# emiliofidalgo/liodom

Hardware: AMD Instinct MI355X
Metric: scans/sec (64×1800 cloud, prev_frames=20) at 1 GPU; pose RMSE vs CPU ref (higher is better)
Workload: dtype f64

## Files before the change

liodom_amd/api.py:

```python
import ctypes as C
import hashlib
import os
import subprocess

import numpy as np

_HERE = os.path.dirname(os.path.abspath(__file__))
_ROOT = os.path.dirname(_HERE)
_LIB = os.path.join(_HERE, "lib", "libliodom_hip.so")
_HASH = _LIB + ".srchash"
_BUILD_INFO = {"rebuilt": None, "source_hash": None}
_SRC = [os.path.join(_HERE, "csrc", f) for f in ("liodom_hip.hip", "liodom_kernels.h", "kernels_extract.h", "kernels_sync.h",
                                                  "kernels_compact.h", "kernels_knn.h", "kernels_knn8.h", "kernels_lm.h", "kernels_rebuild.h",
                                                  "kernels_filter.h", "kernels_cov.h", "kernels_state.h", "liodom_math.h", "wave_ops.h",
                                                  "liodom_map.h", "liodom_map_host.h")] + [
    os.path.join(_ROOT, "include", "liodom_hip.h")]

HIPCC_FLAGS = ["--offload-arch=gfx950", "-O3", "-std=c++17", "-ffp-contract=off", "-fPIC", "-shared",
               "-Wno-unused-value"]


class LiodomError(RuntimeError):
    pass


def lib_path():
    return _LIB


def source_hash():
    h = hashlib.sha256()
    h.update(" ".join(HIPCC_FLAGS).encode())
    for p in _SRC:
        with open(p, "rb") as f:
            h.update(b"\0" + os.path.basename(p).encode() + b"\0" + f.read())
    return h.hexdigest()


def built_hash():
    try:
        with open(_HASH) as f:
            return f.read().strip()
    except OSError:
        return ""


def is_stale():
    return not os.path.exists(_LIB) or built_hash() != source_hash()


def build(force=False, verbose=False):
    import fcntl
    os.makedirs(os.path.dirname(_LIB), exist_ok=True)
    with open(_LIB + ".lock", "w") as lock:
        fcntl.flock(lock, fcntl.LOCK_EX)
        want = source_hash()
        if not force and os.path.exists(_LIB) and built_hash() == want:
            _BUILD_INFO.update(rebuilt=False, source_hash=want)
            return _LIB
        hipcc = "/opt/rocm/bin/hipcc" if os.path.exists("/opt/rocm/bin/hipcc") else "hipcc"
        tmp = _LIB + ".tmp.%d" % os.getpid()
        cmd = [hipcc] + HIPCC_FLAGS + ["-o", tmp, _SRC[0]]
        if verbose:
            print(" ".join(cmd))
        try:
            subprocess.check_call(cmd)
            os.replace(tmp, _LIB)
        finally:
            if os.path.exists(tmp):
                os.remove(tmp)
        with open(_HASH, "w") as f:
            f.write(want + "\n")
        _BUILD_INFO.update(rebuilt=True, source_hash=want)
    return _LIB


def build_info():
    return dict(_BUILD_INFO)


class Params(C.Structure):
    _fields_ = [
        ("min_range", C.c_double), ("max_range", C.c_double),
        ("lidar_type", C.c_int32), ("scan_lines", C.c_int32), ("scan_regions", C.c_int32),
        ("edges_per_region", C.c_int32),
        ("min_points_per_scan", C.c_uint64), ("local_map_size", C.c_uint64),
        ("save_results", C.c_int32),
        ("results_dir", C.c_char * 256), ("fixed_frame", C.c_char * 64), ("base_frame", C.c_char * 64),
        ("laser_frame", C.c_char * 64),
        ("use_imu", C.c_int32), ("filter_local_map", C.c_int32), ("mapping", C.c_int32), ("publish_tf", C.c_int32),
    ]


class Config(C.Structure):
    _fields_ = [
        ("device", C.c_int32), ("n_streams", C.c_int32), ("max_points", C.c_int32), ("max_width", C.c_int32),
        ("reserved1", C.c_int32), ("lm_apply_step_on_ftol", C.c_int32), ("pose_log_capacity", C.c_int32),
# ... 683 lines not shown
```

liodom_amd/csrc/kernels_lm.h:

```cpp
constexpr int kLmWaves = kLmThreads / 64;
__host__ __device__ __forceinline__ size_t lm_lds_bytes(int edge_cap) {
  return (size_t)((edge_cap + 3) & ~3) * sizeof(int);
}


__device__ int lm_compact_bits(const DevView& v, int s, int outer_it, int E, int* idx ) {
  const int lane = threadIdx.x & 63;
  const int Q = v.knn_queries;
  const int nb = (E + Q - 1) / Q;
  const int nwords = (nb + 3) >> 2;
  const unsigned int* mw = reinterpret_cast<const unsigned int*>(v.corr_mask + ((size_t)s * 2 + outer_it) * v.mask_stride);
  int run = 0;
  for (int w0 = 0; w0 < nwords; w0 += 64) {
    const int w = w0 + lane;
    unsigned int word = (w < nwords) ? mw[w] : 0u;
    const int pop = __popc(word);
    const int incl = wave_incl_scan_i32(pop);
    int o = run + incl - pop;
    while (word) {
      const int b = __ffs(word) - 1;
      word &= word - 1u;
      const int bit = w * 32 + b;
      idx[o++] = (bit >> 3) * Q + (bit & 7);
    }
// ... 245 lines not shown
  __hip_atomic_store((gu64*)(base + lane), ((unsigned long long)tag << 32) | word, __ATOMIC_RELAXED, __HIP_MEMORY_SCOPE_AGENT);
}

template <bool kList = false>
__global__ void k_imu_override(DevView v, int s0, int count) {
  const int i = blockIdx.x * blockDim.x + threadIdx.x;
  if (i >= count) return;
  const int s = stream_of_lane<kList>(v, s0, i);
  StreamState& st = v.state[s];
  if (!st.initialized) return;
  double odom[12], out[12], l2b[12], q[4];
#pragma unroll
  for (int k = 0; k < 12; k++) { odom[k] = st.odom[k]; l2b[k] = v.laser_to_base[k]; }
#pragma unroll
  for (int k = 0; k < 4; k++) q[k] = v.imu_q[(size_t)s * 4 + k];
  imu_override(odom, q, l2b, v.rotation_mode, out);
#pragma unroll
  for (int k = 0; k < 12; k++) st.odom[k] = out[k];
  quat_from_pose(out, v.rotation_mode, st.param_q);
  st.param_t[0] = out[3]; st.param_t[1] = out[7]; st.param_t[2] = out[11];
}

__device__ __forceinline__ void pose_cov_store(const DevView& v, int s, const StreamState& st, const LmState& lm, const double* acc, int nblocks, int tid) {
  const int j = tid - 64;
  if (j < 0 || j >= 21) return;
  PoseCovRaw* r = v.cov_raw + s;
  bool applied = lm.termination == LM_TERM_FUNC_TOL && lm.apply_on_ftol != 0;
  for (int k = 0; k < 4; k++) applied = applied && lm.q[k] == lm.cand_q[k];
  for (int k = 0; k < 3; k++) applied = applied && lm.t[k] == lm.cand_t[k];
  r->H[j] = applied ? acc[7 + j] : lm.H[j];
  if (j == 0) {
    r->scan_index = st.info.scan_index; r->n_res = nblocks; r->termination = lm.termination; r->has_solve = 1;
    r->cost = lm.cost;
  }
}

__device__ __forceinline__ void rebuild_beside_solve(const DevView& v, int s, StreamState& st, int eb, int outer_it, int block, int nblocks, unsigned int seq, int* sbase, int* sslot);

template <int kOuterIt, bool kChainMode, bool kList = false>
#ifndef LIODOM_LM_WAVES_PER_SIMD
#define LIODOM_LM_WAVES_PER_SIMD 1
#endif
__global__ __launch_bounds__(kLmThreads, LIODOM_LM_WAVES_PER_SIMD) void k_lm_solve(DevView v, int s0, int eb, unsigned int seq, unsigned int done_target) {
  constexpr int outer_it = kOuterIt;
  constexpr int chain = kChainMode ? 1 : 0;
  __shared__ double sh_pose2[2][12];
  __shared__ int sh_pi, sh_ci;
  __shared__ int sh_nmoved;
  __shared__ double sh_pred_s[20];
  __shared__ int sh_unapplied;
  __shared__ double sh_acc[kAccN];
  __shared__ LmState lm;
  __shared__ int sh_flag;
  __shared__ int sh_C;
  const int s = stream_of<kList>(v, s0, (int)blockIdx.y);
#if defined(LIODOM_CHAIN_PRIO)
  if (v.n_streams <= 4) __builtin_amdgcn_s_setprio(LIODOM_CHAIN_PRIO);
#endif
  const int G = v.lm_groups, gstride = G > 1 ? 8 : 1, bxl = (int)blockIdx.x;
  const bool is_solver = bxl < G * gstride && (bxl % gstride) == 0;
  const int g = is_solver ? bxl / gstride : G + (bxl < G * gstride ? bxl - (bxl / gstride + 1) : bxl - G);
  StreamState& st = v.state[s];
  __shared__ int sh_cnt[kMaxFrames + 1];
  OV_STAMP(v, bxl == 0 && threadIdx.x == 0, outer_it == 0 ? 0 : 3);
  if (seq && outer_it == 0 && bxl == 0 && threadIdx.x == 0) {
    typedef __attribute__((address_space(1))) unsigned int gu32;
    __hip_atomic_store((gu32*)(v.ov_flags + s), seq, __ATOMIC_RELAXED, __HIP_MEMORY_SCOPE_AGENT);
  }
  if (g >= G) {
    if (!v.early_rebuild || chain) return;
    __shared__ int sh_slot[kMaxFrames];
    rebuild_beside_solve(v, s, st, eb, outer_it, g - G, (int)gridDim.x - G, seq, sh_cnt, sh_slot);
    return;
  }
  __shared__ double sh_wsum[kLmWaves][32];
  __shared__ double sh_red[16][32];
  __shared__ double sh_x0[8];
  __shared__ double sh_prev[12];
  __shared__ int sh_fc;
  if (threadIdx.x < 4) sh_x0[threadIdx.x] = st.param_q[threadIdx.x];
  else if (threadIdx.x < 7) sh_x0[threadIdx.x] = st.param_t[threadIdx.x - 4];
  else if (threadIdx.x >= 64 && threadIdx.x < 76) sh_prev[threadIdx.x - 64] = st.prev_odom[threadIdx.x - 64];
  else if (threadIdx.x == 76) sh_fc = st.frame_count;
  __shared__ int sh_spec_at;
  if (threadIdx.x == 77) sh_spec_at = st.spec_eval[outer_it];
  __shared__ int sh_redo;
  if (threadIdx.x == 78) sh_redo = st.spec_redo[outer_it == 0 ? 1 : 0];
  extern __shared__ __attribute__((aligned(16))) int sh_idx[];
  const int tid = threadIdx.x;
  const bool prep = tid < kLmCtl;
  bool dead = false;
  if (chain && outer_it == 0) dead = !chain_wait_count(v.knn_done0 + s, done_target, &st.status);
  if (chain && outer_it == 0 && sh_redo) __builtin_amdgcn_fence(__ATOMIC_ACQUIRE, "agent");
  int E_in;
  if (chain && outer_it == 0) {
    typedef __attribute__((address_space(1))) unsigned int gu32;
    E_in = (int)__hip_atomic_load((gu32*)(v.edge_cnt + eb * 32 + s), __ATOMIC_RELAXED, __HIP_MEMORY_SCOPE_AGENT);
  } else {
    E_in = st.n_edges_buf[eb];
  }
  if (outer_it == 0 && tid == 0 && g == 0) {
    st.info.n_edges = E_in;
    st.info.map_points = st.n_search;
    for (int k = 0; k < 2; k++) {
      st.info.lm[k].iterations = 0; st.info.lm[k].accepted = 0; st.info.lm[k].termination = LM_TERM_NO_RESIDUALS;
      st.info.lm[k].pad = 0; st.info.lm[k].initial_cost = 0.0; st.info.lm[k].final_cost = 0.0;
    }
  }
  if (!st.initialized) {
    if (outer_it == 1 && g == 0) {
      if (seq) ov_wait_knn_done(v, s, seq, &st.status);
      if (tid == 0) st.append_raw = 1;
      __shared__ double sh_T0[12];
      if (tid < 12) sh_T0[tid] = st.odom[tid];
      __syncthreads();
      finalize_scan(v, s, st, sh_cnt, eb, true, 0, 0, sh_T0, 1, true, sh_prev, sh_fc);
      if (tid == 0) st.initialized = 1;
      if (v.cov_raw && tid == 64) {
        PoseCovRaw* r = v.cov_raw + s;
        r->scan_index = st.info.scan_index; r->n_res = 0; r->termination = st.info.lm[1].termination; r->has_solve = 0; r->cost = st.info.lm[1].final_cost;
      }
    }
    return;
  }
  bool clr_pending = outer_it == 1 && g == 0 && prep && !v.early_rebuild;
  auto clear_hash_slots = [&]() {
    hash_clear_used(v, s, st.n_used_tab[0], tid, kLmCtl);
    clr_pending = false;
  };
  const bool dbgb = (s == 0) && (g == 0) && (tid == kLmCtl) && (outer_it == 1);
  const bool dbge = (s == 0) && (g == 0) && (tid == 0) && (outer_it == 1);
  DBG_STAMP(v, dbgb, 2, 0);
  const int E = E_in;
  int nblocks = st.info.matches[outer_it];
  __shared__ int sh_nmatch;
  __shared__ double sh_scale[8];
  const unsigned int epoch0 = ((unsigned int)(st.scan_counter + 1) << 6) | ((unsigned int)outer_it << 5);
  unsigned int n_eval = 0;
  bool xch_local = false;
  LmCache cache;
  int c_lo = 0, c_hi = 0;
  int dbg_it = 0;
  auto evaluate = [&](const double* pose) {
    lm_eval(v, s, outer_it, eb, c_lo, c_hi, sh_idx, pose, &sh_wsum[0][0], cache);
    if (tid >= kLmCtl) {
      const int lane = tid - kLmCtl;
      if (G > 1) {
        const double x = lm_wave_total(&sh_wsum[0][0], c_hi - c_lo, lane >> 1);
        DBG_STAMP(v, dbgb && dbg_it < 4, 2, 12 + dbg_it);
        xch_local = lm_exchange(v, s, g, G, epoch0 | ++n_eval, x, sh_acc, &st.status, xch_local, lane);
      } else {
        if (lane < kAccN) sh_acc[lane] = lm_wave_total(&sh_wsum[0][0], c_hi - c_lo, lane);
        ++n_eval;
      }
      asm volatile("s_waitcnt lgkmcnt(0)" ::: "memory");
      __builtin_amdgcn_wave_barrier();
    }
  };
  auto my_share = [&](int C) {
    const int chunk = (C + G - 1) / G;
    c_lo = g * chunk < C ? g * chunk : C;
    c_hi = (g + 1) * chunk < C ? (g + 1) * chunk : C;
  };
  if (seq && outer_it == 1) { if (chain) dead = !chain_wait_count(v.knn_done0 + 32 + s, done_target, &st.status) || dead; else ov_wait_knn_done(v, s, seq, &st.status); }
  if (seq && outer_it == 1) { __syncthreads(); if (sh_redo) __builtin_amdgcn_fence(__ATOMIC_ACQUIRE, "agent"); }
  OV_STAMP(v, g == 0 && tid == 0 && outer_it == 1, 4);
  OV_STAMP(v, g == 0 && tid == 0 && outer_it == 0, 18);
  if (v.knn_partials) {
    const int Q = v.knn_queries;
    const int nb = (E + Q - 1) / Q;
    const double* part = v.knn_part + ((size_t)s * 2 + outer_it) * v.knn_blocks * 32;
    constexpr int kRC = kLmThreads / 32;
    const int i = tid & 31, r0 = tid >> 5;
    double x0 = 0.0, x1 = 0.0;
    if (i <= kAccN) {
      const int nb_cap = v.knn_blocks;
      for (int rb = r0; rb < (dead ? 0 : (rb == r0 ? nb_cap : nb)); rb += 16 * kRC) {
        double xs[16];
#pragma unroll
        for (int u = 0; u < 16; u++) { const int r = rb + kRC * u; xs[u] = (r < nb_cap) ? part[(size_t)r * 32 + i] : 0.0; }
#pragma unroll
        for (int u = 0; u < 16; u++) { const int r = rb + kRC * u; if (r >= nb) xs[u] = 0.0; }
#pragma unroll
        for (int u = 0; u < 16; u += 2) { x0 += xs[u]; x1 += xs[u + 1]; }
      }
    }
    sh_red[r0][i] = x0 + x1;
    __syncthreads();
    if (tid <= kAccN) {
      double x = 0.0;
#pragma unroll
      for (int r = 0; r < kRC; r++) x += sh_red[r][tid];
      if (tid < kAccN) sh_acc[tid] = x;
      else { sh_nmatch = (int)x; if (g == 0) st.info.matches[outer_it] = (int)x; }
    }
    __syncthreads();
    nblocks = sh_nmatch;
  } else {
    __syncthreads();
    if (prep) {
      const int C = lm_compact_bits(v, s, outer_it, E, sh_idx);
      if (tid == 0) sh_C = C;
    } else if (tid == kLmCtl) {
      iso_from_qt(sh_x0, sh_x0 + 4, sh_pose2[0]);
    }
    __syncthreads();
    my_share(sh_C);
    lm_cache_load(v, s, outer_it, eb, c_lo, c_hi, sh_idx, cache);
    evaluate(sh_pose2[0]);
  }
  DBG_STAMP(v, dbgb, 2, 2);
  int pi = 0, ci = -1, nmoved = 0;
  const unsigned int n_eval0 = n_eval;
  const bool spec_ok = v.speculate != 0 && v.speculate != 5 && v.speculate != 7 && g == 0 && seq != 0u && outer_it == 0;
  const bool spec_ok1 = v.speculate != 0 && v.speculate != 4 && v.speculate != 6 && g == 0 && chain != 0 && outer_it == 1 && v.early_rebuild && v.pred_xch != nullptr;
  const bool spec_forced = v.speculate == 2 || v.speculate == 6 || v.speculate == 7;
  bool spec_done = false;
  int spec_moves = -1;
  for (int step = 0;; step++) {
    if (step == 0 && tid > kLmCtl && tid <= kLmCtl + 6) {
      const int j = tid - kLmCtl - 1;
      sh_scale[j] = 1.0 / (1.0 + sqrt(sh_acc[7 + h_idx(j, j)]));
    }
    if (step == 0) __builtin_amdgcn_wave_barrier();
    if (tid == kLmCtl) {
      const int acc_before = step == 0 ? 0 : lm.accepted;
      const int f = step == 0 ? lm_begin(lm, sh_x0, sh_x0 + 4, sh_acc, nblocks, v.apply_on_ftol, sh_scale) : lm_update(lm, sh_acc);
      sh_flag = f;
      bool moved = step > 0 && lm.accepted != acc_before;
      if (step > 0 && !moved && f != LM_NEED_EVAL && lm.termination == LM_TERM_FUNC_TOL) {
        moved = true;
        for (int k = 0; k < 4; k++) moved = moved && lm.q[k] == lm.cand_q[k];
        for (int k = 0; k < 3; k++) moved = moved && lm.t[k] == lm.cand_t[k];
      }
      if (moved) { ci = pi; pi ^= 1; nmoved++; }
      if (f == LM_NEED_EVAL) iso_from_qt(lm.cand_q, lm.cand_t, sh_pose2[pi]);
      sh_pi = pi; sh_ci = ci; sh_nmoved = nmoved; sh_unapplied = (step > 0 && !moved) ? 1 : 0;
      if (step == 0) DBG_STAMP(v, dbgb, 2, 23);
    } else if (!prep) {
    } else if (step == 0 && v.knn_partials) {
      DBG_STAMP(v, dbge, 2, 24);
      const int C = dead ? 0 : lm_compact_bits(v, s, outer_it, E, sh_idx);
      if (tid == 0) sh_C = C;
      DBG_STAMP(v, dbge, 2, 25);
      my_share(C);
      lm_cache_load(v, s, outer_it, eb, c_lo, c_hi, sh_idx, cache);
    } else if (clr_pending) {
      clear_hash_slots();
    }
    __syncthreads();
    if (step == 0) { if (v.knn_partials && !prep) my_share(sh_C); DBG_STAMP(v, dbgb, 2, 3); }
    else { DBG_STAMP(v, dbgb && dbg_it < 5, 2, 5 + 2 * dbg_it); dbg_it++; }
    if (sh_flag != LM_NEED_EVAL) break;
    if ((spec_ok || spec_ok1) && !spec_done && sh_ci >= 0 &&
        (spec_forced || (!spec_forced && sh_spec_at == 0 && lm.model_cost_change <= v.spec_theta * 1e-6 * lm.cost))) {
      if (spec_ok) {
        ov_publish_pose(v, s, sh_pose2[sh_ci], &lm.q[0], seq, tid, 1);
        OV_STAMP(v, tid == 0, 19);
      } else if (tid >= kLmCtl) {
        const int l = tid - kLmCtl;
        if (l < 25) publish_final_pose(v, s, sh_pose2[sh_ci], 0, (unsigned int)sh_fc + 1u, l, 0);
        if (l == 0) predict_next(sh_pose2[sh_ci], sh_prev, v.rotation_mode, sh_pred_s);
        asm volatile("s_waitcnt lgkmcnt(0)" ::: "memory");
        __builtin_amdgcn_wave_barrier();
        pred_publish(v, s, sh_pred_s, (unsigned int)sh_fc + 1u, l, 64, 1);
        OV_STAMP(v, l == 0, 22);
      }
      if ((kInstrument && (v.debug & 64)) && tid == 0) atomicAdd(&v.dbg_clk[270], 1ull);
      spec_done = true;
      spec_moves = sh_nmoved;
    }
    const double* pose_c = sh_pose2[sh_pi];
    evaluate(pose_c);
    DBG_STAMP(v, dbgb && dbg_it < 5, 2, 4 + 2 * dbg_it);
  }
  if (clr_pending) clear_hash_slots();
  DBG_STAMP(v, dbgb, 2, 20);
  if ((kInstrument && (v.debug & 32)) && dbgb) v.dbg_clk[2 * 32 + 27] = (xch_local ? 100ull : 0ull) + 10ull * xcc_id() + (unsigned long long)n_eval;
  if (g != 0) return;
  __shared__ double sh_ov[20];
  __shared__ liodom_lm_trace_t sh_trace;
  {
    if (tid == kLmCtl) {
      sh_trace.iterations = lm.iter; sh_trace.accepted = lm.accepted; sh_trace.termination = lm.termination; sh_trace.pad = 0;
      sh_trace.initial_cost = lm.initial_cost; sh_trace.final_cost = lm.cost;
    }
    const int cif = sh_ci;
    if (cif >= 0) {
      if (tid < 12) sh_ov[tid] = sh_pose2[cif][tid];
      else if (tid >= 64 && tid < 71) sh_ov[12 + tid - 64] = (&lm.q[0])[tid - 64];
    } else if (tid == kLmCtl) {
      double q[4], t[3], T[12];
      for (int k = 0; k < 4; k++) q[k] = lm.q[k];
      for (int k = 0; k < 3; k++) t[k] = lm.t[k];
      iso_from_qt(q, t, T);
      for (int k = 0; k < 12; k++) sh_ov[k] = T[k];
      for (int k = 0; k < 4; k++) sh_ov[12 + k] = q[k];
      for (int k = 0; k < 3; k++) sh_ov[16 + k] = t[k];
    }
  }
  __syncthreads();
  if (outer_it == 0) {
    if (seq) { ov_publish_pose(v, s, sh_ov, sh_ov + 12, seq, tid, spec_done ? 2 : 3); OV_STAMP(v, tid == 0, 1); }
  } else if (v.early_rebuild && tid < 50) {
    if (tid >= 25 || !spec_done) publish_final_pose(v, s, sh_ov, 0, (unsigned int)sh_fc + 1u, tid % 25, tid / 25);
  }
  if (tid == kLmCtl) {
    if (outer_it == 0) {
      for (int k = 0; k < 4; k++) st.param_q[k] = sh_ov[12 + k];
      for (int k = 0; k < 3; k++) st.param_t[k] = sh_ov[16 + k];
      for (int k = 0; k < 12; k++) st.odom[k] = sh_ov[k];
    }
    st.spec_eval[outer_it] = (spec_done && sh_nmoved != spec_moves) ? v.spec_backoff : (sh_spec_at > 0 ? sh_spec_at - 1 : 0);
    st.spec_redo[outer_it] = (spec_done && sh_nmoved != spec_moves) ? 1 : 0;
    if (spec_done) { st.spec_stats[2 * outer_it] += 1; if (sh_nmoved != spec_moves) st.spec_stats[2 * outer_it + 1] += 1; }
    if (outer_it == 0) st.info.lm[0] = sh_trace;
    if (outer_it == 1) st.append_raw = 0;
  }
  DBG_STAMP(v, dbgb, 2, 21);
  if (outer_it == 1) {
    finalize_scan(v, s, st, sh_cnt, eb, false, kLmCtl, chain, sh_ov, 0, false, sh_prev, sh_fc, spec_done ? 2 : 3, (!spec_done || sh_nmoved == spec_moves) ? 1u : 2u, &sh_trace);
    if (v.cov_raw) pose_cov_store(v, s, st, lm, sh_acc, nblocks, tid);
    DBG_STAMP(v, dbgb, 2, 22);
  }
  DBG_STAMP(v, dbgb, 2, 28);
  OV_STAMP(v, tid == 0, outer_it == 0 ? 2 : 5);
}
```

liodom_amd/csrc/liodom_kernels.h:

```cpp
#pragma once
#include <hip/hip_runtime.h>

#include <cstddef>

#include "../../include/liodom_hip.h"
#include "liodom_math.h"
#include "wave_ops.h"

namespace liodom_dev {

#ifndef LIODOM_CHAIN_PRIO
#define LIODOM_CHAIN_PRIO 2
#endif
constexpr int kWave = 64;
constexpr uint64_t kEmptyKey = 0xFFFFFFFFFFFFFFFFull;
#ifndef LIODOM_LM_THREADS
#define LIODOM_LM_THREADS 256
#endif
constexpr int kLmThreads = LIODOM_LM_THREADS;
constexpr int kLmEvalThreads = kLmThreads;
constexpr int kLmCtl = kLmThreads - 64;
#ifndef LIODOM_LM_GROUPS_MAX
#define LIODOM_LM_GROUPS_MAX 8
#endif
constexpr int kLmGroupsMax = LIODOM_LM_GROUPS_MAX;
constexpr int kKnnGroup = 32;
constexpr int kMaxFrames = 256;
constexpr int kEdgeBufs = 4;
constexpr int kEdgePipeBufs = 3;
constexpr int kEdgeBufX = 3;
constexpr int kOvReplicas = 8;
constexpr int kOvGranules = 38;
constexpr int kPredGranules = 38;
constexpr int kStreamLists = 2 * kEdgePipeBufs;
constexpr int kStreamListBase = 64;
constexpr int kStreamListChunk = 256;

struct StreamState {
  double odom[12];
  double prev_odom[12];
  double final_odom[12];
  double param_q[4];
  double param_t[3];
  int32_t initialized;
  int32_t append_raw;
  int32_t frame_count;
  int32_t n_frames;
  int32_t n_edges_buf[4];
  int32_t reb_frame_count;
  int32_t n_map;
  int32_t n_used_tab[2];
  int32_t cursor;
  int32_t scan_counter;
  uint32_t status;
  int32_t n_search;
  uint32_t table_mask;
  int32_t n_filt;
  int32_t vox_used;
  int32_t vox_cursor;
  int32_t vox_minb[3];
  int32_t vox_divb[3];
  int32_t n_recv;
  int32_t n_ovf[2];
  int32_t reb_initialized;
  int32_t reb_pad;
  int32_t spec_eval[2];
  int32_t hb_main_fc;
  int32_t hb_main_old;
  int32_t hb_main_nf;
  int32_t hb_base[8];
  int32_t hb_shift;
  int32_t hb_cursor;
  int32_t hb_stats[4];
  int32_t hb_spill;
  int32_t spec_redo[2];
  int32_t spec_stats[4];
  double pred_odom[2][12];
  liodom_step_info_t info;
};

struct __attribute__((aligned(16))) CellSlot {
  unsigned long long key;
  unsigned int start;
  unsigned int cnt;
};

#define LD_TAB_PARITY(v, frame_count) ((v).early_rebuild ? ((frame_count) & 1) : 0)

struct HostOut {
  double pose[7];
// ... 227 lines not shown
```

liodom_amd/csrc/liodom_math.h:

```cpp
#pragma once
#include <cfloat>
#include <cmath>
#include <cstdint>

#if defined(__HIPCC__)
#define LD_HD __host__ __device__ __forceinline__
#define LD_UNROLL _Pragma("unroll")
#define LD_FP_CONTRACT_FAST _Pragma("clang fp contract(fast)")
#else
#define LD_HD inline
#define LD_UNROLL
#define LD_FP_CONTRACT_FAST
#endif
#if defined(__HIP_DEVICE_COMPILE__)
#define LD_RSQRT(x) rsqrt(x)
#else
#define LD_RSQRT(x) (1.0 / sqrt(x))
#endif

namespace liodom_dev {

constexpr int kJacobiSweeps = 8;
constexpr int kLmMaxIterations = 4;
constexpr double kHuberA = 0.2;
// ... 632 lines not shown
      n2 += x * x;
      if (fabs(x) > fabs(big)) big = x;
    }
    const double sc = (big < 0.0 ? -1.0 : 1.0) / sqrt(n2);
    LD_UNROLL
    for (int k = 0; k < 6; k++) evecs[k * 6 + r] = V[k * 6 + o] * sc;
  }
  return sweep;
}

LD_HD unsigned int pose_cov_compute(const double* H21, double final_cost, int n_res, int termination, int has_solve,
                                    double* sigma2, double* info36, double* cov36, double* evals6, double* evecs36) {
  const double nan = __builtin_nan("");
  LD_UNROLL
  for (int i = 0; i < 36; i++) { info36[i] = nan; cov36[i] = nan; evecs36[i] = nan; }
  LD_UNROLL
  for (int i = 0; i < 6; i++) evals6[i] = nan;
  *sigma2 = nan;
  if (!has_solve) return kCovNoSolve;
  if (termination == LM_TERM_EVAL_FAILURE) return kCovEvalFailure;
  unsigned int flags = 0u;
  bool finite = true;
  LD_UNROLL
  for (int i = 0; i < 21; i++) finite = finite && ld_isfinite(H21[i]);
  if (n_res > 0 && finite && ld_isfinite(final_cost)) flags |= kCovValid;
  if (3 * n_res <= 6) flags |= kCovFewResiduals;
  else *sigma2 = 2.0 * final_cost / (double)(3 * n_res - 6);
  if (!finite) return flags | kCovSingular;
  LD_UNROLL
  for (int i = 0; i < 6; i++) {
    LD_UNROLL
    for (int j = 0; j < 6; j++) info36[i * 6 + j] = h_at(H21, i, j);
  }
  sym_eig6(info36, evals6, evecs36);
  double inv[36];
  if (!spd_inverse6(H21, inv)) return flags | kCovSingular;
  if ((flags & kCovValid) && !(flags & kCovFewResiduals)) {
    LD_UNROLL
    for (int i = 0; i < 36; i++) cov36[i] = *sigma2 * inv[i];
  }
  return flags;
}

LD_HD void pose_cov_to_ros(const double* cov36_tangent, const double* T12, const double* L12, double* out36) {
  double u[3];
  LD_UNROLL
  for (int i = 0; i < 3; i++) u[i] = T12[4 * i] * L12[3] + T12[4 * i + 1] * L12[7] + T12[4 * i + 2] * L12[11];
  double A[36];
  LD_UNROLL
  for (int i = 0; i < 36; i++) A[i] = 0.0;
  A[0 * 6 + 1] = 2.0 * u[2];  A[0 * 6 + 2] = -2.0 * u[1];
  A[1 * 6 + 0] = -2.0 * u[2]; A[1 * 6 + 2] = 2.0 * u[0];
  A[2 * 6 + 0] = 2.0 * u[1];  A[2 * 6 + 1] = -2.0 * u[0];
  LD_UNROLL
  for (int i = 0; i < 3; i++) { A[i * 6 + 3 + i] = 1.0; A[(3 + i) * 6 + i] = 2.0; }
  double AS[36];
  LD_UNROLL
  for (int i = 0; i < 6; i++) {
    LD_UNROLL
    for (int j = 0; j < 6; j++) {
      double s = 0.0;
      LD_UNROLL
      for (int k = 0; k < 6; k++) s += A[i * 6 + k] * cov36_tangent[k * 6 + j];
      AS[i * 6 + j] = s;
    }
  }
  LD_UNROLL
  for (int i = 0; i < 6; i++) {
    LD_UNROLL
    for (int j = 0; j < 6; j++) {
      double s = 0.0;
      LD_UNROLL
      for (int k = 0; k < 6; k++) s += AS[i * 6 + k] * A[j * 6 + k];
      out36[i * 6 + j] = s;
    }
  }
}

LD_HD double norm7(const double* q, const double* t) {
  LD_FP_CONTRACT_FAST
  return sqrt(q[0] * q[0] + q[1] * q[1] + q[2] * q[2] + q[3] * q[3] + t[0] * t[0] + t[1] * t[1] + t[2] * t[2]);
}

LD_HD int lm_propose(LmState& st) {
  LD_FP_CONTRACT_FAST
  while (true) {
    if (st.iter >= kLmMaxIterations) { st.termination = LM_TERM_MAX_ITER; return LM_DONE; }
    if (st.radius < 1e-32) { st.termination = LM_TERM_RADIUS; return LM_DONE; }
    st.iter++;
    double sc[6], gs[6];
    LD_UNROLL
    for (int i = 0; i < 6; i++) { sc[i] = st.scale[i]; gs[i] = sc[i] * st.g[i]; }
    double A[21];
    LD_UNROLL
    for (int i = 0; i < 6; i++) {
      LD_UNROLL
      for (int j = 0; j <= i; j++) A[lt_idx(i, j)] = sc[i] * sc[j] * st.H[h_idx(j, i)];
    }
    if (!st.reuse_diagonal) {
      LD_UNROLL
      for (int j = 0; j < 6; j++) {
        double d = A[lt_idx(j, j)];
        if (d < 1e-6) d = 1e-6;
        if (d > 1e32) d = 1e32;
        st.diag[j] = d;
      }
    }
    const double inv_radius = 1.0 / st.radius;
    LD_UNROLL
    for (int j = 0; j < 6; j++) A[lt_idx(j, j)] += st.diag[j] * inv_radius;
    double y[6];
    const bool ok = chol_solve6_packed(A, gs, y);
    st.reuse_diagonal = 1;
    double mcc = 0.0;
    double step[6];
    if (ok) {
      double sg = 0.0, shs = 0.0;
      LD_UNROLL
      for (int i = 0; i < 6; i++) step[i] = -y[i];
      LD_UNROLL
      for (int i = 0; i < 6; i++) {
        sg += step[i] * gs[i];
        double row = 0.0;
        LD_UNROLL
        for (int j = 0; j < i; j++) row += (sc[i] * sc[j] * st.H[h_idx(j, i)]) * step[j];
        shs += step[i] * (2.0 * row + (sc[i] * sc[i] * st.H[h_idx(i, i)]) * step[i]);
      }
      mcc = -sg - 0.5 * shs;
    }
    if (!ok || !(mcc > 0.0)) {
      if (++st.invalid_run >= 5) { st.termination = LM_TERM_INVALID_STEPS; return LM_DONE; }
      st.radius = st.radius * 0.5;
      continue;
    }
    st.invalid_run = 0;
    st.model_cost_change = mcc;
    double delta[6];
    LD_UNROLL
    for (int j = 0; j < 6; j++) delta[j] = step[j] * sc[j];
    quat_plus(st.q, delta, st.cand_q);
    LD_UNROLL
    for (int k = 0; k < 3; k++) st.cand_t[k] = st.t[k] + delta[3 + k];
    return LM_NEED_EVAL;
  }
}

LD_HD int lm_begin(LmState& st, const double* q0, const double* t0, const double* acc,
                   int n_blocks, int apply_on_ftol, const double* pre_scale = nullptr) {
  LD_UNROLL
  for (int k = 0; k < 4; k++) st.q[k] = st.cand_q[k] = q0[k];
  LD_UNROLL
  for (int k = 0; k < 3; k++) st.t[k] = st.cand_t[k] = t0[k];
  st.iter = 0; st.accepted = 0; st.invalid_run = 0; st.termination = LM_TERM_MAX_ITER;
  st.apply_on_ftol = apply_on_ftol;
  st.cost = 0.0; st.initial_cost = 0.0; st.model_cost_change = 0.0;
  st.radius = 1e4; st.decrease_factor = 2.0; st.reuse_diagonal = 0;
  LD_UNROLL
  for (int j = 0; j < 6; j++) { st.scale[j] = 1.0; st.diag[j] = 0.0; st.g[j] = 0.0; }
  LD_UNROLL
  for (int j = 0; j < 21; j++) st.H[j] = 0.0;
  st.x_norm = norm7(st.q, st.t);
  if (n_blocks == 0) { st.termination = LM_TERM_NO_RESIDUALS; return LM_DONE; }
  if (acc[28] != 0.0) { st.termination = LM_TERM_EVAL_FAILURE; return LM_DONE; }
  st.cost = acc[0]; st.initial_cost = acc[0];
  double gmax = 0.0;
  LD_UNROLL
  for (int j = 0; j < 6; j++) { st.g[j] = acc[1 + j]; const double ag = fabs(st.g[j]); if (ag > gmax) gmax = ag; }
  LD_UNROLL
  for (int j = 0; j < 21; j++) st.H[j] = acc[7 + j];
  LD_UNROLL
  for (int j = 0; j < 6; j++) st.scale[j] = pre_scale ? pre_scale[j] : 1.0 / (1.0 + sqrt(st.H[h_idx(j, j)]));
  if (gmax <= 1e-10) { st.termination = LM_TERM_GRAD_TOL; return LM_DONE; }
  return lm_propose(st);
}

LD_HD int lm_update(LmState& st, const double* acc) {
  LD_FP_CONTRACT_FAST
  const double cand_cost = (acc[28] != 0.0) ? DBL_MAX : acc[0];
  double dq[4], dt[3];
  LD_UNROLL
  for (int k = 0; k < 4; k++) dq[k] = st.q[k] - st.cand_q[k];
  LD_UNROLL
  for (int k = 0; k < 3; k++) dt[k] = st.t[k] - st.cand_t[k];
  const double step_sq = dq[0] * dq[0] + dq[1] * dq[1] + dq[2] * dq[2] + dq[3] * dq[3] + dt[0] * dt[0] + dt[1] * dt[1] + dt[2] * dt[2];
  const double ptol = 1e-8 * (st.x_norm + 1e-8);
  const double ptol_sq = ptol * ptol;
  bool ptol_hit = step_sq <= ptol_sq * (1.0 - 1e-12);
  if (!ptol_hit && step_sq <= ptol_sq * (1.0 + 1e-12)) ptol_hit = sqrt(step_sq) <= ptol;
  if (ptol_hit) { st.termination = LM_TERM_PARAM_TOL; return LM_DONE; }
  const double cost_change = st.cost - cand_cost;
  if (fabs(cost_change) <= 1e-6 * st.cost) {
    st.termination = LM_TERM_FUNC_TOL;
    if (st.apply_on_ftol && cost_change > 0.0) {
      LD_UNROLL
      for (int k = 0; k < 4; k++) st.q[k] = st.cand_q[k];
      LD_UNROLL
      for (int k = 0; k < 3; k++) st.t[k] = st.cand_t[k];
      st.cost = cand_cost;
    }
    return LM_DONE;
  }
  const double rel = cost_change / st.model_cost_change;
  if (rel > 1e-3) {
    LD_UNROLL
    for (int k = 0; k < 4; k++) st.q[k] = st.cand_q[k];
    LD_UNROLL
    for (int k = 0; k < 3; k++) st.t[k] = st.cand_t[k];
    st.x_norm = norm7(st.q, st.t);
    st.cost = cand_cost;
    double gmax = 0.0;
    LD_UNROLL
    for (int j = 0; j < 6; j++) { st.g[j] = acc[1 + j]; const double ag = fabs(st.g[j]); if (ag > gmax) gmax = ag; }
    LD_UNROLL
    for (int j = 0; j < 21; j++) st.H[j] = acc[7 + j];
    st.accepted++;
    const double c = 2.0 * rel - 1.0;
    double f = 1.0 - c * c * c;
    if (f < 1.0 / 3.0) f = 1.0 / 3.0;
    st.radius = st.radius / f;
    if (st.radius > 1e16) st.radius = 1e16;
    st.decrease_factor = 2.0;
    st.reuse_diagonal = 0;
    if (gmax <= 1e-10) { st.termination = LM_TERM_GRAD_TOL; return LM_DONE; }
  } else {
    st.radius = st.radius / st.decrease_factor;
    st.decrease_factor *= 2.0;
    st.reuse_diagonal = 1;
  }
  return lm_propose(st);
}

}
```

Before: 14920.

## Spread LM control-step bookkeeping across the control wave's lanes

Replaces the single-lane Levenberg-Marquardt begin/update/propose logic with wave-cooperative versions. Lanes now prepare the state, form the scaled Hessian and gradient, copy the gradient and Hessian, and run a DPP max reduction in parallel, and the state is initialised early while the KNN wait is still pending. The x_norm recompute is deferred until just before the evaluate call. This aims to shorten the serial control-lane critical path between evaluations, at the cost of extra wave syncs and more complex shared LM state handling.

```diff
diff --git a/liodom_amd/api.py b/liodom_amd/api.py
--- a/liodom_amd/api.py
+++ b/liodom_amd/api.py
@@ -12,7 +12,7 @@
 _BUILD_INFO = {"rebuilt": None, "source_hash": None}
 _SRC = [os.path.join(_HERE, "csrc", f) for f in ("liodom_hip.hip", "liodom_kernels.h", "kernels_extract.h", "kernels_sync.h",
                                                   "kernels_compact.h", "kernels_knn.h", "kernels_knn8.h", "kernels_lm.h", "kernels_rebuild.h",
-                                                  "kernels_filter.h", "kernels_cov.h", "kernels_state.h", "liodom_math.h", "wave_ops.h",
+                                                  "kernels_filter.h", "kernels_cov.h", "kernels_state.h", "liodom_math.h", "wave_ops.h", "lm_ctl_wave.h",
                                                   "liodom_map.h", "liodom_map_host.h")] + [
     os.path.join(_ROOT, "include", "liodom_hip.h")]
 
diff --git a/liodom_amd/csrc/kernels_lm.h b/liodom_amd/csrc/kernels_lm.h
--- a/liodom_amd/csrc/kernels_lm.h
+++ b/liodom_amd/csrc/kernels_lm.h
@@ -351,6 +351,14 @@
   else if (threadIdx.x < 7) sh_x0[threadIdx.x] = st.param_t[threadIdx.x - 4];
   else if (threadIdx.x >= 64 && threadIdx.x < 76) sh_prev[threadIdx.x - 64] = st.prev_odom[threadIdx.x - 64];
   else if (threadIdx.x == 76) sh_fc = st.frame_count;
+  __shared__ LmWaveScratch sh_ws;
+  double ctl_x0 = 0.0;
+  if (threadIdx.x >= kLmCtl && threadIdx.x < kLmCtl + 7) { const int k = (int)threadIdx.x - kLmCtl; ctl_x0 = k < 4 ? st.param_q[k] : st.param_t[k - 4]; }
+  bool ctl_prepared = false;
+  auto ctl_prepare = [&]() {
+    if (threadIdx.x >= kLmCtl && !ctl_prepared) lm_wave_prepare(lm, sh_ws, ctl_x0, v.apply_on_ftol, (int)threadIdx.x - kLmCtl);
+    ctl_prepared = true;
+  };
   __shared__ int sh_spec_at;
   if (threadIdx.x == 77) sh_spec_at = st.spec_eval[outer_it];
   __shared__ int sh_redo;
@@ -359,6 +367,7 @@
   const int tid = threadIdx.x;
   const bool prep = tid < kLmCtl;
   bool dead = false;
+  if (chain && outer_it == 0) ctl_prepare();
   if (chain && outer_it == 0) dead = !chain_wait_count(v.knn_done0 + s, done_target, &st.status);
   if (chain && outer_it == 0 && sh_redo) __builtin_amdgcn_fence(__ATOMIC_ACQUIRE, "agent");
   int E_in;
@@ -403,7 +412,6 @@
   const int E = E_in;
   int nblocks = st.info.matches[outer_it];
   __shared__ int sh_nmatch;
-  __shared__ double sh_scale[8];
   const unsigned int epoch0 = ((unsigned int)(st.scan_counter + 1) << 6) | ((unsigned int)outer_it << 5);
   unsigned int n_eval = 0;
   bool xch_local = false;
@@ -431,6 +439,7 @@
     c_lo = g * chunk < C ? g * chunk : C;
     c_hi = (g + 1) * chunk < C ? (g + 1) * chunk : C;
   };
+  if (seq && outer_it == 1) ctl_prepare();
   if (seq && outer_it == 1) { if (chain) dead = !chain_wait_count(v.knn_done0 + 32 + s, done_target, &st.status) || dead; else ov_wait_knn_done(v, s, seq, &st.status); }
   if (seq && outer_it == 1) { __syncthreads(); if (sh_redo) __builtin_amdgcn_fence(__ATOMIC_ACQUIRE, "agent"); }
   OV_STAMP(v, g == 0 && tid == 0 && outer_it == 1, 4);
@@ -456,6 +465,7 @@
     }
     sh_red[r0][i] = x0 + x1;
     __syncthreads();
+    ctl_prepare();
     if (tid <= kAccN) {
       double x = 0.0;
 #pragma unroll
@@ -470,8 +480,9 @@
     if (prep) {
       const int C = lm_compact_bits(v, s, outer_it, E, sh_idx);
       if (tid == 0) sh_C = C;
-    } else if (tid == kLmCtl) {
-      iso_from_qt(sh_x0, sh_x0 + 4, sh_pose2[0]);
+    } else {
+      ctl_prepare();
+      if (tid == kLmCtl) iso_from_qt(sh_x0, sh_x0 + 4, sh_pose2[0]);
     }
     __syncthreads();
     my_share(sh_C);
@@ -487,26 +498,22 @@
   bool spec_done = false;
   int spec_moves = -1;
   for (int step = 0;; step++) {
-    if (step == 0 && tid > kLmCtl && tid <= kLmCtl + 6) {
-      const int j = tid - kLmCtl - 1;
-      sh_scale[j] = 1.0 / (1.0 + sqrt(sh_acc[7 + h_idx(j, j)]));
-    }
-    if (step == 0) __builtin_amdgcn_wave_barrier();
-    if (tid == kLmCtl) {
-      const int acc_before = step == 0 ? 0 : lm.accepted;
-      const int f = step == 0 ? lm_begin(lm, sh_x0, sh_x0 + 4, sh_acc, nblocks, v.apply_on_ftol, sh_scale) : lm_update(lm, sh_acc);
-      sh_flag = f;
-      bool moved = step > 0 && lm.accepted != acc_before;
-      if (step > 0 && !moved && f != LM_NEED_EVAL && lm.termination == LM_TERM_FUNC_TOL) {
-        moved = true;
-        for (int k = 0; k < 4; k++) moved = moved && lm.q[k] == lm.cand_q[k];
-        for (int k = 0; k < 3; k++) moved = moved && lm.t[k] == lm.cand_t[k];
-      }
-      if (moved) { ci = pi; pi ^= 1; nmoved++; }
-      if (f == LM_NEED_EVAL) iso_from_qt(lm.cand_q, lm.cand_t, sh_pose2[pi]);
-      sh_pi = pi; sh_ci = ci; sh_nmoved = nmoved; sh_unapplied = (step > 0 && !moved) ? 1 : 0;
-      if (step == 0) DBG_STAMP(v, dbgb, 2, 23);
-    } else if (!prep) {
+    if (!prep) {
+      const int acc_before = step == 0 ? 0 : __builtin_amdgcn_readfirstlane(lm.accepted);
+      const int f = step == 0 ? lm_wave_begin(lm, sh_ws, sh_acc, nblocks, tid - kLmCtl) : lm_wave_update(lm, sh_ws, sh_acc, tid - kLmCtl);
+      if (tid == kLmCtl) {
+        sh_flag = f;
+        bool moved = step > 0 && lm.accepted != acc_before;
+        if (step > 0 && !moved && f != LM_NEED_EVAL && lm.termination == LM_TERM_FUNC_TOL) {
+          moved = true;
+          for (int k = 0; k < 4; k++) moved = moved && lm.q[k] == lm.cand_q[k];
+          for (int k = 0; k < 3; k++) moved = moved && lm.t[k] == lm.cand_t[k];
+        }
+        if (moved) { ci = pi; pi ^= 1; nmoved++; }
+        if (f == LM_NEED_EVAL) iso_from_qt(lm.cand_q, lm.cand_t, sh_pose2[pi]);
+        sh_pi = pi; sh_ci = ci; sh_nmoved = nmoved; sh_unapplied = (step > 0 && !moved) ? 1 : 0;
+        if (step == 0) DBG_STAMP(v, dbgb, 2, 23);
+      }
     } else if (step == 0 && v.knn_partials) {
       DBG_STAMP(v, dbge, 2, 24);
       const int C = dead ? 0 : lm_compact_bits(v, s, outer_it, E, sh_idx);
@@ -540,6 +547,7 @@
       spec_moves = sh_nmoved;
     }
     const double* pose_c = sh_pose2[sh_pi];
+    if (!prep) lm_wave_deferred(lm, sh_ws, tid - kLmCtl);
     evaluate(pose_c);
     DBG_STAMP(v, dbgb && dbg_it < 5, 2, 4 + 2 * dbg_it);
   }
diff --git a/liodom_amd/csrc/liodom_kernels.h b/liodom_amd/csrc/liodom_kernels.h
--- a/liodom_amd/csrc/liodom_kernels.h
+++ b/liodom_amd/csrc/liodom_kernels.h
@@ -6,6 +6,7 @@
 #include "../../include/liodom_hip.h"
 #include "liodom_math.h"
 #include "wave_ops.h"
+#include "lm_ctl_wave.h"
 
 namespace liodom_dev {
 
diff --git a/liodom_amd/csrc/liodom_math.h b/liodom_amd/csrc/liodom_math.h
--- a/liodom_amd/csrc/liodom_math.h
+++ b/liodom_amd/csrc/liodom_math.h
@@ -738,71 +738,104 @@
   return sqrt(q[0] * q[0] + q[1] * q[1] + q[2] * q[2] + q[3] * q[3] + t[0] * t[0] + t[1] * t[1] + t[2] * t[2]);
 }
 
+LD_HD int lt_row(int e) { return (e >= 1) + (e >= 3) + (e >= 6) + (e >= 10) + (e >= 15); }
+LD_HD double lm_scaled_entry(const double* scale, const double* H, int i, int j) {
+  LD_FP_CONTRACT_FAST
+  return scale[i] * scale[j] * H[h_idx(j, i)];
+}
+LD_HD double lm_scaled_grad(const double* scale, const double* g, int i) { return scale[i] * g[i]; }
+LD_HD double lm_diag_clamp(double d) {
+  if (d < 1e-6) d = 1e-6;
+  if (d > 1e32) d = 1e32;
+  return d;
+}
+LD_HD double lm_damped(double a, double diag, double inv_radius) {
+  LD_FP_CONTRACT_FAST
+  return a + diag * inv_radius;
+}
+LD_HD double lm_row_quad(const double* ar, const double* step, int i) {
+  LD_FP_CONTRACT_FAST
+  double row = 0.0;
+  LD_UNROLL
+  for (int j = 0; j < 5; j++) { if (j < i) row += ar[j] * step[j]; }
+  return 2.0 * row + ar[i] * step[i];
+}
+LD_HD double lm_gabs(double g) { const double a = fabs(g); return a == a ? a : 0.0; }
+LD_HD double lm_jacobi_scale(double hjj) { return 1.0 / (1.0 + sqrt(hjj)); }
+LD_HD double lm_delta(double step, double scale) { return step * scale; }
+LD_HD double lm_cand_t(double t, double step, double scale) {
+  LD_FP_CONTRACT_FAST
+  return t + step * scale;
+}
+
+LD_HD bool lm_invalid_step(LmState& st) {
+  if (++st.invalid_run >= 5) { st.termination = LM_TERM_INVALID_STEPS; return false; }
+  st.radius = st.radius * 0.5;
+  return true;
+}
+
+LD_HD bool lm_solve_step(LmState& st, const double* A0 , const double* gs ) {
+  LD_FP_CONTRACT_FAST
+  double A[21];
+  LD_UNROLL
+  for (int e = 0; e < 21; e++) A[e] = A0[e];
+  const double inv_radius = 1.0 / st.radius;
+  LD_UNROLL
+  for (int j = 0; j < 6; j++) A[lt_idx(j, j)] = lm_damped(A[lt_idx(j, j)], st.diag[j], inv_radius);
+  double y[6];
+  const bool ok = chol_solve6_packed(A, gs, y);
+  st.reuse_diagonal = 1;
+  if (!ok) return false;
+  double step[6];
+  double sg = 0.0, shs = 0.0;
+  LD_UNROLL
+  for (int i = 0; i < 6; i++) step[i] = -y[i];
+  LD_UNROLL
+  for (int i = 0; i < 6; i++) {
+    sg += step[i] * gs[i];
+    shs += step[i] * lm_row_quad(A0 + lt_idx(i, 0), step, i);
+  }
+  const double mcc = -sg - 0.5 * shs;
+  if (!(mcc > 0.0)) return false;
+  st.invalid_run = 0;
+  st.model_cost_change = mcc;
+  double delta[3];
+  LD_UNROLL
+  for (int j = 0; j < 3; j++) delta[j] = lm_delta(step[j], st.scale[j]);
+  quat_plus(st.q, delta, st.cand_q);
+  LD_UNROLL
+  for (int k = 0; k < 3; k++) st.cand_t[k] = lm_cand_t(st.t[k], step[3 + k], st.scale[3 + k]);
+  return true;
+}
+
 LD_HD int lm_propose(LmState& st) {
   LD_FP_CONTRACT_FAST
+  double A0[21], gs[6];
+  bool formed = false;
   while (true) {
     if (st.iter >= kLmMaxIterations) { st.termination = LM_TERM_MAX_ITER; return LM_DONE; }
     if (st.radius < 1e-32) { st.termination = LM_TERM_RADIUS; return LM_DONE; }
     st.iter++;
-    double sc[6], gs[6];
-    LD_UNROLL
-    for (int i = 0; i < 6; i++) { sc[i] = st.scale[i]; gs[i] = sc[i] * st.g[i]; }
-    double A[21];
-    LD_UNROLL
-    for (int i = 0; i < 6; i++) {
-      LD_UNROLL
-      for (int j = 0; j <= i; j++) A[lt_idx(i, j)] = sc[i] * sc[j] * st.H[h_idx(j, i)];
-    }
-    if (!st.reuse_diagonal) {
-      LD_UNROLL
-      for (int j = 0; j < 6; j++) {
-        double d = A[lt_idx(j, j)];
-        if (d < 1e-6) d = 1e-6;
-        if (d > 1e32) d = 1e32;
-        st.diag[j] = d;
+    if (!formed) {
+      LD_UNROLL
+      for (int i = 0; i < 6; i++) gs[i] = lm_scaled_grad(st.scale, st.g, i);
+      LD_UNROLL
+      for (int i = 0; i < 6; i++) {
+        LD_UNROLL
+        for (int j = 0; j <= i; j++) A0[lt_idx(i, j)] = lm_scaled_entry(st.scale, st.H, i, j);
       }
-    }
-    const double inv_radius = 1.0 / st.radius;
-    LD_UNROLL
-    for (int j = 0; j < 6; j++) A[lt_idx(j, j)] += st.diag[j] * inv_radius;
-    double y[6];
-    const bool ok = chol_solve6_packed(A, gs, y);
-    st.reuse_diagonal = 1;
-    double mcc = 0.0;
-    double step[6];
-    if (ok) {
-      double sg = 0.0, shs = 0.0;
-      LD_UNROLL
-      for (int i = 0; i < 6; i++) step[i] = -y[i];
-      LD_UNROLL
-      for (int i = 0; i < 6; i++) {
-        sg += step[i] * gs[i];
-        double row = 0.0;
+      if (!st.reuse_diagonal) {
         LD_UNROLL
-        for (int j = 0; j < i; j++) row += (sc[i] * sc[j] * st.H[h_idx(j, i)]) * step[j];
-        shs += step[i] * (2.0 * row + (sc[i] * sc[i] * st.H[h_idx(i, i)]) * step[i]);
+        for (int j = 0; j < 6; j++) st.diag[j] = lm_diag_clamp(A0[lt_idx(j, j)]);
       }
-      mcc = -sg - 0.5 * shs;
-    }
-    if (!ok || !(mcc > 0.0)) {
-      if (++st.invalid_run >= 5) { st.termination = LM_TERM_INVALID_STEPS; return LM_DONE; }
-      st.radius = st.radius * 0.5;
-      continue;
-    }
-    st.invalid_run = 0;
-    st.model_cost_change = mcc;
-    double delta[6];
-    LD_UNROLL
-    for (int j = 0; j < 6; j++) delta[j] = step[j] * sc[j];
-    quat_plus(st.q, delta, st.cand_q);
-    LD_UNROLL
-    for (int k = 0; k < 3; k++) st.cand_t[k] = st.t[k] + delta[3 + k];
-    return LM_NEED_EVAL;
-  }
-}
-
-LD_HD int lm_begin(LmState& st, const double* q0, const double* t0, const double* acc,
-                   int n_blocks, int apply_on_ftol, const double* pre_scale = nullptr) {
+      formed = true;
+    }
+    if (lm_solve_step(st, A0, gs)) return LM_NEED_EVAL;
+    if (!lm_invalid_step(st)) return LM_DONE;
+  }
+}
+
+LD_HD void lm_begin_prepare(LmState& st, const double* q0, const double* t0, int apply_on_ftol) {
   LD_UNROLL
   for (int k = 0; k < 4; k++) st.q[k] = st.cand_q[k] = q0[k];
   LD_UNROLL
@@ -816,21 +849,27 @@
   LD_UNROLL
   for (int j = 0; j < 21; j++) st.H[j] = 0.0;
   st.x_norm = norm7(st.q, st.t);
+}
+
+LD_HD int lm_begin(LmState& st, const double* q0, const double* t0, const double* acc,
+                   int n_blocks, int apply_on_ftol, const double* pre_scale = nullptr) {
+  lm_begin_prepare(st, q0, t0, apply_on_ftol);
   if (n_blocks == 0) { st.termination = LM_TERM_NO_RESIDUALS; return LM_DONE; }
   if (acc[28] != 0.0) { st.termination = LM_TERM_EVAL_FAILURE; return LM_DONE; }
   st.cost = acc[0]; st.initial_cost = acc[0];
   double gmax = 0.0;
   LD_UNROLL
-  for (int j = 0; j < 6; j++) { st.g[j] = acc[1 + j]; const double ag = fabs(st.g[j]); if (ag > gmax) gmax = ag; }
+  for (int j = 0; j < 6; j++) { st.g[j] = acc[1 + j]; const double ag = lm_gabs(st.g[j]); if (ag > gmax) gmax = ag; }
   LD_UNROLL
   for (int j = 0; j < 21; j++) st.H[j] = acc[7 + j];
   LD_UNROLL
-  for (int j = 0; j < 6; j++) st.scale[j] = pre_scale ? pre_scale[j] : 1.0 / (1.0 + sqrt(st.H[h_idx(j, j)]));
+  for (int j = 0; j < 6; j++) st.scale[j] = pre_scale ? pre_scale[j] : lm_jacobi_scale(st.H[h_idx(j, j)]);
   if (gmax <= 1e-10) { st.termination = LM_TERM_GRAD_TOL; return LM_DONE; }
   return lm_propose(st);
 }
 
-LD_HD int lm_update(LmState& st, const double* acc) {
+enum { LM_STEP_DONE = 0, LM_STEP_ACCEPTED = 1, LM_STEP_REJECTED = 2 };
+LD_HD int lm_decide(LmState& st, const double* acc) {
   LD_FP_CONTRACT_FAST
   const double cand_cost = (acc[28] != 0.0) ? DBL_MAX : acc[0];
   double dq[4], dt[3];
@@ -843,7 +882,7 @@
   const double ptol_sq = ptol * ptol;
   bool ptol_hit = step_sq <= ptol_sq * (1.0 - 1e-12);
   if (!ptol_hit && step_sq <= ptol_sq * (1.0 + 1e-12)) ptol_hit = sqrt(step_sq) <= ptol;
-  if (ptol_hit) { st.termination = LM_TERM_PARAM_TOL; return LM_DONE; }
+  if (ptol_hit) { st.termination = LM_TERM_PARAM_TOL; return LM_STEP_DONE; }
   const double cost_change = st.cost - cand_cost;
   if (fabs(cost_change) <= 1e-6 * st.cost) {
     st.termination = LM_TERM_FUNC_TOL;
@@ -854,21 +893,11 @@
       for (int k = 0; k < 3; k++) st.t[k] = st.cand_t[k];
       st.cost = cand_cost;
     }
-    return LM_DONE;
+    return LM_STEP_DONE;
   }
   const double rel = cost_change / st.model_cost_change;
   if (rel > 1e-3) {
-    LD_UNROLL
-    for (int k = 0; k < 4; k++) st.q[k] = st.cand_q[k];
-    LD_UNROLL
-    for (int k = 0; k < 3; k++) st.t[k] = st.cand_t[k];
-    st.x_norm = norm7(st.q, st.t);
     st.cost = cand_cost;
-    double gmax = 0.0;
-    LD_UNROLL
-    for (int j = 0; j < 6; j++) { st.g[j] = acc[1 + j]; const double ag = fabs(st.g[j]); if (ag > gmax) gmax = ag; }
-    LD_UNROLL
-    for (int j = 0; j < 21; j++) st.H[j] = acc[7 + j];
     st.accepted++;
     const double c = 2.0 * rel - 1.0;
     double f = 1.0 - c * c * c;
@@ -877,11 +906,29 @@
     if (st.radius > 1e16) st.radius = 1e16;
     st.decrease_factor = 2.0;
     st.reuse_diagonal = 0;
+    return LM_STEP_ACCEPTED;
+  }
+  st.radius = st.radius / st.decrease_factor;
+  st.decrease_factor *= 2.0;
+  st.reuse_diagonal = 1;
+  return LM_STEP_REJECTED;
+}
+
+LD_HD int lm_update(LmState& st, const double* acc) {
+  const int d = lm_decide(st, acc);
+  if (d == LM_STEP_DONE) return LM_DONE;
+  if (d == LM_STEP_ACCEPTED) {
+    LD_UNROLL
+    for (int k = 0; k < 4; k++) st.q[k] = st.cand_q[k];
+    LD_UNROLL
+    for (int k = 0; k < 3; k++) st.t[k] = st.cand_t[k];
+    st.x_norm = norm7(st.q, st.t);
+    double gmax = 0.0;
+    LD_UNROLL
+    for (int j = 0; j < 6; j++) { st.g[j] = acc[1 + j]; const double ag = lm_gabs(st.g[j]); if (ag > gmax) gmax = ag; }
+    LD_UNROLL
+    for (int j = 0; j < 21; j++) st.H[j] = acc[7 + j];
     if (gmax <= 1e-10) { st.termination = LM_TERM_GRAD_TOL; return LM_DONE; }
-  } else {
-    st.radius = st.radius / st.decrease_factor;
-    st.decrease_factor *= 2.0;
-    st.reuse_diagonal = 1;
   }
   return lm_propose(st);
 }
diff --git a/liodom_amd/csrc/lm_ctl_wave.h b/liodom_amd/csrc/lm_ctl_wave.h
--- /dev/null
+++ b/liodom_amd/csrc/lm_ctl_wave.h
@@ -0,0 +1,126 @@
+#pragma once
+#include <cstddef>
+#include "liodom_math.h"
+#include "wave_ops.h"
+
+namespace liodom_dev {
+
+struct LmWaveScratch {
+  double A[21];
+  double gs[6];
+  int xnorm_pending;
+};
+
+static_assert(offsetof(LmState, cand_t) == 11 * sizeof(double) && offsetof(LmState, H) == offsetof(LmState, g) + 6 * sizeof(double),
+              "LmState: q t cand_q cand_t and g H are contiguous runs of doubles");
+static_assert(offsetof(LmWaveScratch, gs) == 21 * sizeof(double), "LmWaveScratch: gs follows A");
+
+__device__ __forceinline__ void lm_wave_sync() {
+  asm volatile("s_waitcnt lgkmcnt(0)" ::: "memory");
+  __builtin_amdgcn_wave_barrier();
+}
+__device__ __forceinline__ bool lm_wave_lane0(bool b) { return __builtin_amdgcn_readfirstlane((int)b) != 0; }
+
+__device__ __forceinline__ void lm_wave_prepare(LmState& st, LmWaveScratch& ws, double x0, int apply_on_ftol, int lane) {
+  double* pt = &st.q[0];
+  if (lane < 7) { pt[lane] = x0; pt[7 + lane] = x0; }
+  if (lane < 27) (&st.g[0])[lane] = 0.0;
+  else if (lane < 33) st.scale[lane - 27] = 1.0;
+  else if (lane < 39) st.diag[lane - 33] = 0.0;
+  if (lane == 0) {
+    st.iter = 0; st.accepted = 0; st.invalid_run = 0; st.termination = LM_TERM_MAX_ITER;
+    st.apply_on_ftol = apply_on_ftol;
+    st.cost = 0.0; st.initial_cost = 0.0; st.model_cost_change = 0.0;
+    st.radius = 1e4; st.decrease_factor = 2.0; st.reuse_diagonal = 0;
+    ws.xnorm_pending = 0;
+  }
+  lm_wave_sync();
+  if (lane == 0) st.x_norm = norm7(st.q, st.t);
+  lm_wave_sync();
+}
+
+__device__ __forceinline__ int lm_wave_propose(LmState& st, LmWaveScratch& ws, int lane) {
+  bool formed = false;
+  while (true) {
+    if (__builtin_amdgcn_readfirstlane(st.iter) >= kLmMaxIterations) { if (lane == 0) st.termination = LM_TERM_MAX_ITER; lm_wave_sync(); return LM_DONE; }
+    if (lm_wave_lane0(st.radius < 1e-32)) { if (lane == 0) st.termination = LM_TERM_RADIUS; lm_wave_sync(); return LM_DONE; }
+    if (!formed) {
+      if (lane < 21) {
+        const int i = lt_row(lane), j = lane - lt_idx(i, 0);
+        const double a = lm_scaled_entry(st.scale, st.H, i, j);
+        ws.A[lane] = a;
+        if (i == j && !st.reuse_diagonal) st.diag[j] = lm_diag_clamp(a);
+      } else if (lane < 27) {
+        (&ws.A[0])[lane] = lm_scaled_grad(st.scale, st.g, lane - 21);
+      }
+      formed = true;
+      lm_wave_sync();
+    }
+    bool again = false;
+    int f = LM_NEED_EVAL;
+    if (lane == 0) {
+      st.iter++;
+      if (!lm_solve_step(st, ws.A, ws.gs)) { again = lm_invalid_step(st); f = LM_DONE; }
+    }
+    lm_wave_sync();
+    if (!lm_wave_lane0(again)) return __builtin_amdgcn_readfirstlane(f);
+  }
+}
+
+__device__ __forceinline__ int lm_wave_begin(LmState& st, LmWaveScratch& ws, const double* acc, int n_blocks, int lane) {
+  if (n_blocks == 0) { if (lane == 0) st.termination = LM_TERM_NO_RESIDUALS; lm_wave_sync(); return LM_DONE; }
+  if (lm_wave_lane0(acc[28] != 0.0)) { if (lane == 0) st.termination = LM_TERM_EVAL_FAILURE; lm_wave_sync(); return LM_DONE; }
+  double ag = 0.0;
+  if (lane < 27) {
+    const double x = acc[1 + lane];
+    (&st.g[0])[lane] = x;
+    if (lane < 6) ag = lm_gabs(x);
+  } else if (lane >= 32 && lane < 38) {
+    const int j = lane - 32;
+    st.scale[j] = lm_jacobi_scale(acc[7 + h_idx(j, j)]);
+  } else if (lane == 40) {
+    const double c = acc[0];
+    st.cost = c; st.initial_cost = c;
+  }
+  ag = fmax(ag, dpp_f64<DPP_XOR1>(ag));
+  ag = fmax(ag, dpp_f64<DPP_XOR2>(ag));
+  ag = fmax(ag, dpp_f64<DPP_HALF_MIRROR>(ag));
+  lm_wave_sync();
+  if (lm_wave_lane0(ag <= 1e-10)) { if (lane == 0) st.termination = LM_TERM_GRAD_TOL; lm_wave_sync(); return LM_DONE; }
+  return lm_wave_propose(st, ws, lane);
+}
+
+__device__ __forceinline__ int lm_wave_update(LmState& st, LmWaveScratch& ws, const double* acc, int lane) {
+  int d = LM_STEP_DONE;
+  if (lane == 0) d = lm_decide(st, acc);
+  d = __builtin_amdgcn_readfirstlane(d);
+  if (d == LM_STEP_DONE) { lm_wave_sync(); return LM_DONE; }
+  if (d == LM_STEP_ACCEPTED) {
+    double ag = 0.0;
+    if (lane < 27) {
+      const double x = acc[1 + lane];
+      (&st.g[0])[lane] = x;
+      if (lane < 6) ag = lm_gabs(x);
+    } else if (lane >= 32 && lane < 39) {
+      double* pt = &st.q[0];
+      pt[lane - 32] = pt[7 + lane - 32];
+    } else if (lane == 40) {
+      ws.xnorm_pending = 1;
+    }
+    ag = fmax(ag, dpp_f64<DPP_XOR1>(ag));
+    ag = fmax(ag, dpp_f64<DPP_XOR2>(ag));
+    ag = fmax(ag, dpp_f64<DPP_HALF_MIRROR>(ag));
+    lm_wave_sync();
+    if (lm_wave_lane0(ag <= 1e-10)) { if (lane == 0) st.termination = LM_TERM_GRAD_TOL; lm_wave_sync(); return LM_DONE; }
+  }
+  return lm_wave_propose(st, ws, lane);
+}
+
+__device__ __forceinline__ void lm_wave_deferred(LmState& st, LmWaveScratch& ws, int lane) {
+  if (__builtin_amdgcn_readfirstlane(ws.xnorm_pending)) {
+    if (lane == 0) { st.x_norm = norm7(st.q, st.t); ws.xnorm_pending = 0; }
+    lm_wave_sync();
+  }
+}
+
+}
```

Measured after the change: 14800. No clear change (-0.8%).
